# JiaoXianjun/multi-rtl-sdr-calibration

Hardware: AMD Instinct MI355X
Metric: IQ Msamples/s through FCCH+SCH calib (higher is better)
Workload: dtype f64; 1 GPU; cfg4 full chain gsm_sync_demod.m:107-124: 64 dongle streams (64/GPU) x 1020000 IQ samples (102 frames), fir1(46), FCCH+SCH+total_ppm_calculation, table on the host; streams_per_gpu=64, streams_total=64, output=table, collective=none, rows_checked_vs_oracle_per_rank=0

## Files before the change

### multi-rtl-sdr-calibration_amd/csrc/abi_calls.h

```cpp
#pragma once

const char* gsmcal_version(void) { return GSMCAL_VERSION; }

void gsmcal_params_default(gsmcal_params* p) {
    if (!p) return;
    p->coarse_th_db = 10.0; p->coarse_mv_factor = 10; p->coarse_max_offset = 5; p->min_hits = 5;
    p->fine_max_offset = 64; p->fine_max_ppm = 4000.0; p->fine_gate_snr_db = 5.0; p->fine_noise_bw_hz = 200e3;
    p->sch_max_offset = 8; p->sch_max_ppm = 400.0; p->post_min_bcch = 4;
    p->scan_min_hits = 3; p->scan_spacing = 12500.0; p->scan_spacing_idle = 12500.0 + 1250.0; p->scan_tol = 50.0;
}

int gsmcal_set_params(gsmcal_ctx* c, const gsmcal_params* p) {
    if (!c || !p) return GSMCAL_E_ARG;
    RET_IF(pipe_join(c));
    gsmcal_params d;
    gsmcal_params_default(&d);
    if (p->coarse_mv_factor != d.coarse_mv_factor || p->coarse_max_offset != d.coarse_max_offset ||
        p->fine_max_offset != d.fine_max_offset || p->fine_noise_bw_hz != d.fine_noise_bw_hz || p->sch_max_offset != d.sch_max_offset) {
        c->err = "gsmcal_set_params: a geometry field differs from its default";
        return GSMCAL_E_UNSUPPORTED;
    }
    if (p->min_hits < 2 || p->min_hits > GSMCAL_MAX_HITS || p->scan_min_hits < 1 || p->post_min_bcch < 0) {
        c->err = "gsmcal_set_params: min_hits outside 2..GSMCAL_MAX_HITS, scan_min_hits < 1 or post_min_bcch < 0";
        return GSMCAL_E_ARG;
// ... 41 lines not shown
    (void)hipFuncSetAttribute((const void*)k_burst_tone<1, 0, 0>, hipFuncAttributeMaxDynamicSharedMemorySize, 159 * 1024);
    (void)hipFuncSetAttribute((const void*)k_window_sch<0, 0, 0>, hipFuncAttributeMaxDynamicSharedMemorySize, 159 * 1024);
    (void)hipFuncSetAttribute((const void*)k_post_chain_r<0, 0, 0>, hipFuncAttributeMaxDynamicSharedMemorySize, 159 * 1024);
    (void)hipFuncSetAttribute((const void*)k_post_chain_r<8, 512, 47>, hipFuncAttributeMaxDynamicSharedMemorySize, 159 * 1024);
    (void)hipFuncSetAttribute((const void*)k_sch_equalise, hipFuncAttributeMaxDynamicSharedMemorySize, 159 * 1024);
    (void)hipFuncSetAttribute((const void*)k_sch_fd_training, hipFuncAttributeMaxDynamicSharedMemorySize, 159 * 1024);
    (void)hipFuncSetAttribute((const void*)k_fcch_demod, hipFuncAttributeMaxDynamicSharedMemorySize, 159 * 1024);
    (void)hipFuncSetAttribute((const void*)k_fft_burst<0>, hipFuncAttributeMaxDynamicSharedMemorySize, 159 * 1024);
    (void)hipFuncSetAttribute((const void*)k_fft_burst<1>, hipFuncAttributeMaxDynamicSharedMemorySize, 159 * 1024);
    (void)hipFuncSetAttribute((const void*)k_burst_tone<0, 8, 47>, hipFuncAttributeMaxDynamicSharedMemorySize, 159 * 1024);
    (void)hipFuncSetAttribute((const void*)k_burst_tone<1, 8, 47>, hipFuncAttributeMaxDynamicSharedMemorySize, 159 * 1024);
    (void)hipFuncSetAttribute((const void*)k_window_sch<8, 512, 47>, hipFuncAttributeMaxDynamicSharedMemorySize, 159 * 1024);
    (void)hipGetLastError();
    gsmcal_ctx* c = new gsmcal_ctx();
    gsmcal_params_default(&c->params);
    c->device = device_id;
    c->stream = (hipStream_t)hip_stream;
    c->own_stream = false;
    c->lanes[0].stream = c->stream;
    c->cur = &c->lanes[0];
    const char* e = getenv("GSMCAL_LANES");
    if (e && atoi(e) >= 1) c->n_lanes_cfg = atoi(e) > MAX_LANES ? MAX_LANES : atoi(e);
    { int ncu = 0; if (hipDeviceGetAttribute(&ncu, hipDeviceAttributeMultiprocessorCount, c->device) == hipSuccess && ncu > 0) c->n_cu = ncu; }
    if (const char* e2 = getenv("GSMCAL_SNR_INLINE_MIN")) c->snr_inline_min = atoi(e2);
    if (const char* e2 = getenv("GSMCAL_SNR_INLINE_KEEP")) c->snr_inline_keep = atoi(e2);
    if (const char* e2 = getenv("GSMCAL_FRONT_NT")) c->front_nt = atoi(e2);
    if (const char* e2 = getenv("GSMCAL_SCAN_SPLIT")) c->scan_split = atoi(e2);
    const char* sst = getenv("GSMCAL_SCAN_STAGES");
    if (sst && atoi(sst) >= 1) c->scan_stages = atoi(sst);
    const char* lm = getenv("GSMCAL_LANE_MIN");
    if (lm && atoi(lm) >= 1) c->lane_min = atoi(lm);
    const char* ce = getenv("GSMCAL_CERT");
    if (ce) c->certify = atoi(ce) != 0;
    const char* sfe = getenv("GSMCAL_SNR_FULL");
    if (sfe) c->snr_full = atoi(sfe) != 0;
    const char* sse = getenv("GSMCAL_SNR_SCREEN_DB");
    if (sse) c->snr_screen_db = atof(sse);
    const char* fge = getenv("GSMCAL_FUSE_GATHER");
    if (fge) c->fuse_fine_gather = atoi(fge) != 0;
    const char* fpe = getenv("GSMCAL_FUSE_POST");
    if (fpe) c->fuse_post = atoi(fpe) != 0;
    const char* pse = getenv("GSMCAL_POST_SLOTS");
    if (pse && atoi(pse) >= 1) c->post_slots_cap = atoi(pse);
    const char* pe = getenv("GSMCAL_PRESCREEN");
    if (pe && atoi(pe) == 0) c->prescreen = false;
    const char* fg = getenv("GSMCAL_FRONT_GENERIC");
// ... 1261 lines not shown
```

### multi-rtl-sdr-calibration_amd/csrc/host_plan.h

```cpp
#pragma once
namespace {

struct DevBuf {
    void* p = nullptr;
    size_t cap = 0;
};

struct ProfRec {
    int name_id;
    hipEvent_t e0, e1;
};

}

#define MAX_LANES 32
struct Lane {
    hipStream_t stream = nullptr;
    DevBuf state, dec, win, peaks, snrbuf, x0, chunkrec, openlist, cert, partial, tailctr, xch, xepoch;
    int npartial = 0;
    hipEvent_t done = nullptr;
    hipEvent_t front_done = nullptr;
    int lo = 0, n = 0;
    long snr_stride = 0, snr_nmove = 0;
    int win_l0_len = 0, win_l0_H = 0;
// ... 8 lines not shown
    Lane lanes[MAX_LANES];
    Lane* cur = nullptr;
    int n_lanes_cfg = 4;
    int n_lanes_used = 1;
    const double* cf_lane = nullptr;
    hipEvent_t fork = nullptr;
    struct GraphSlot {
        std::vector<uintptr_t> key;
        unsigned long epoch = 0;
        int seen = 0;
        hipGraph_t graph = nullptr;
        hipGraphExec_t exec = nullptr;
        unsigned long used = 0;
        int fused_streams = 0;
    };
    static constexpr int GRAPH_SLOTS = 4;
    GraphSlot g_calib[GRAPH_SLOTS], g_scan[GRAPH_SLOTS];
    unsigned long g_stamp = 0;
    unsigned long ws_epoch = 0;
    bool use_graph = true;
    bool graph_always = false;
    bool prescreen = true;
    int n_cu = 256;
    int snr_inline_min = 1;
    int snr_inline_keep = 0;
    int front_nt = -1;
    size_t call_raw_bytes = 0;
    const void* last_raw = nullptr;
    bool call_raw_fresh = false;
    int scan_split = 88;
    int scan_stages = 0;
    int lane_min = 64;
    bool certify = true;
    bool snr_full = true;
    double snr_screen_db = 5.0;
    bool fuse_fine_gather = true;
    static constexpr int FUSED_MAX_STREAMS = 1024;
    std::vector<unsigned> fused_expected;
    unsigned* fused_done = nullptr;
    int fused_hi = 0;
    unsigned long long n_fused_launches = 0, n_gate_fallbacks = 0;
    int capture_fused_streams = 0;
    struct FusedCall {
        const uint8_t* d_raw; int d; long n; int ntaps, len_ts;
        std::vector<double> coef, ts, cf;
        double* d_table; double* d_pos_info; double* d_r_correct; long* d_r_len;
// ... 185 lines not shown
    int kind;
    const uint8_t* raw; long raw_stride;
    const cplx* arr; long arr_stride;
    const double* coef; int ntaps;
};

size_t gather_lds(int len, int level, int kind, int ntaps, bool to_lds = false) {
    return gather_carve(len, level, kind, ntaps, to_lds).total;
}

GatherArgs gather_args(const Source& src, int level, int len) {
    GatherArgs a;
    memset(&a, 0, sizeof(a));
    a.src_kind = src.kind; a.level = level; a.len = len; a.tiles = 0; a.ntaps = src.ntaps;
    a.raw = src.raw; a.raw_stride = src.raw_stride; a.arr = src.arr; a.arr_stride = src.arr_stride;
    a.coef = src.coef;
    return a;
}

size_t fused_lds(const Source& src, int level, int len, size_t scratch, bool compact_xs = false) {
    return (gather_carve(len, level, src.kind, src.ntaps, true, compact_xs).total + scratch + 15) & ~(size_t)15;
}

int launch_gather(gsmcal_ctx* c, int S, const Source& src, int level, int len, bool tiles, int nwin_grid,
                  cplx* dst, long dst_stream_stride, long dst_win_stride) {
    GatherArgs a;
    memset(&a, 0, sizeof(a));
    a.src_kind = src.kind; a.level = level; a.len = len; a.tiles = tiles ? 1 : 0; a.ntaps = src.ntaps; a.pad = 0;
    a.raw = src.raw; a.raw_stride = src.raw_stride; a.arr = src.arr; a.arr_stride = src.arr_stride;
    a.coef = src.coef; a.dst = dst; a.dst_stream_stride = dst_stream_stride; a.dst_win_stride = dst_win_stride;
    const size_t lds = gather_lds(len, level, src.kind, src.ntaps);
    LAUNCH(c, k_gather, dim3(nwin_grid, S), dim3(256), lds, (const StreamState*)c->cur->state.p, a);
    CHECK_LAUNCH(c);
    return 0;
}

int ensure_twiddles(gsmcal_ctx* c, int nfft) {
    if (c->tw_n == nfft) return 0;
    RET_IF(ensure(c, c->tw, (size_t)nfft * sizeof(cplx)));
    LAUNCH(c, k_make_twiddles, dim3((nfft + 255) / 256), dim3(256), 0, (cplx*)c->tw.p, nfft);
    CHECK_LAUNCH(c);
    c->tw_n = nfft;
    ++c->ws_epoch;
    return 0;
}

// ... 279 lines not shown
                return 0;
            }
        }
        TailArgs tl;
        RET_IF(make_tail(c, S, sa_fine, STEP_FINE_DECIDE, lvl, 0, tl));
        LAUNCH(c, k_fine_verify, dim3(H, S), dim3(FV_THREADS), vlds, (const StreamState*)st, (const cplx*)win, sstride, wstride,
               g.fine_nshift, g.nfft, (const cplx*)c->tw.p, (const ChunkRec*)c->cur->chunkrec.p, peaks, H, certp, n_open,
               st, tl);
    } else {
        RET_IF(ensure(c, c->cur->x0, (size_t)S * H * g.nfft * sizeof(cplx)));
        LAUNCH(c, k_fft_burst<1>, dim3(H, S), dim3(FFT_THREADS), fft_lds(g), (const StreamState*)st, (const cplx*)win, sstride,
               wstride, g.nfft, (const cplx*)c->tw.p, (PeakOut*)nullptr, (cplx*)c->cur->x0.p, H);
        LAUNCH(c, k_fine_search, dim3(g.NB, H, S), dim3(256), (size_t)(g.fine_nshift - 1 + FS_CHUNK) * sizeof(cplx),
               (const StreamState*)st, (const cplx*)win, sstride, wstride, g.fine_nshift, g.nfft, (const cplx*)c->cur->x0.p,
               peaks, H, g.NB);
        LAUNCH(c, k_step<STEP_FINE_DECIDE>, dim3(S), dim3(64), 0, st, sa_fine, lvl, 0);
    }
    {
        GatherArgs ga = gather_args(src, lvl + 1, g.nfft);
        if (c->cur->win_l0_len > 0) { ga.l0 = win; ga.l0_stream_stride = sstride; ga.l0_win_stride = wstride; ga.l0_len = c->cur->win_l0_len; }
        TailArgs tl;
        RET_IF(make_tail(c, S, sa, next_sch_lvl >= 0 ? (STEP_CARRIER_DECIDE | STEP_SCH_SETUP) : STEP_CARRIER_DECIDE, lvl,
                         next_sch_lvl >= 0 ? next_sch_lvl : 0, tl));
        LAUNCH_GEOM(g.ov == 8 && src.kind == SRC_RAW && src.ntaps == 47 && lvl == 0, c, (k_burst_tone<1, 8, 47>), (k_burst_tone<1, 0, 0>), dim3(H, S), dim3(BT_THREADS), fused_lds(src, lvl + 1, g.nfft, burst_scratch(g)), st, ga,
               g.nfft, (const cplx*)c->tw.p, g.ov, 1, tl);
    }
    CHECK_LAUNCH(c);
    return 0;
}

int run_sch(gsmcal_ctx* c, int S, const Source& src, int lvl, const Geom& g, int H, int len_ts, bool setup_done,
            int next_post_lvl) {
    StreamState* st = (StreamState*)c->cur->state.p;
    const int wl = g.sch_nshift - 1 + len_ts;
    const long wstride = g.fine_wlen > wl ? g.fine_wlen : wl, sstride = (long)H * wstride;
    RET_IF(ensure(c, c->cur->win, (size_t)S * sstride * sizeof(cplx)));
    const StepArgs sa = step_args(c, g, H, len_ts);
    if (!setup_done) LAUNCH(c, k_step<STEP_SCH_SETUP>, dim3(S), dim3(64), 0, st, sa, 0, lvl);
    {
        const GatherArgs ga = gather_args(src, lvl, wl);
        const size_t scratch = (size_t)(len_ts + g.sch_nshift * SCH_PARTS) * sizeof(cplx) + (size_t)g.sch_nshift * sizeof(double);
        TailArgs tl;
        RET_IF(make_tail(c, S, sa, next_post_lvl >= 0 ? (STEP_SCH_DECIDE | STEP_POST_SETUP) : STEP_SCH_DECIDE, lvl,
                         next_post_lvl >= 0 ? next_post_lvl : 0, tl));
        LAUNCH_GEOM(g.ov == 8 && len_ts == 512 && src.kind == SRC_RAW && src.ntaps == 47 && lvl == 2, c, (k_window_sch<8, 512, 47>), (k_window_sch<0, 0, 0>), dim3(H, S), dim3(512), fused_lds(src, lvl, wl, scratch), st, ga, (const cplx*)c->ts.p,
               len_ts, g.sch_nshift, tl);
    }
    CHECK_LAUNCH(c);
    return 0;
}

int run_post(gsmcal_ctx* c, int S, const Source& src, int lvl, const Geom& g, int H, bool setup_done, double* table,
             double* pos_info_out, long* r_len_out) {
    StreamState* st = (StreamState*)c->cur->state.p;
    const long wstride = g.fine_wlen, sstride = (long)H * g.fine_wlen;
    RET_IF(ensure(c, c->cur->win, (size_t)S * sstride * sizeof(cplx)));
    RET_IF(ensure(c, c->cur->peaks, (size_t)S * H * g.NB * sizeof(PeakOut)));
    RET_IF(ensure_twiddles(c, g.nfft));
    cplx* win = (cplx*)c->cur->win.p;
    StepArgs sa = step_args(c, g, H, 0);
    sa.table = table; sa.pos_info_out = pos_info_out; sa.r_len_out = r_len_out;
    if (!setup_done) LAUNCH(c, k_step<STEP_POST_SETUP>, dim3(S), dim3(64), 0, st, sa, 0, lvl);
    {
        GatherArgs ga = gather_args(src, lvl, g.nfft);
        if (c->cur->win_l0_len == g.fine_wlen && c->cur->win_l0_H == H && src.kind == SRC_RAW) {
            ga.l0 = win; ga.l0_stream_stride = sstride; ga.l0_win_stride = wstride; ga.l0_len = c->cur->win_l0_len;
        }
        TailArgs tl;
        RET_IF(make_tail(c, S, sa, table ? (STEP_POST_DECIDE | STEP_TOTALS) : STEP_POST_DECIDE, lvl, 0, tl));
        LAUNCH_GEOM(g.ov == 8 && src.kind == SRC_RAW && src.ntaps == 47 && lvl == 3, c, (k_burst_tone<0, 8, 47>), (k_burst_tone<0, 0, 0>), dim3(H, S), dim3(BT_THREADS), fused_lds(src, lvl, g.nfft, burst_scratch(g)), st, ga,
               g.nfft, (const cplx*)c->tw.p, g.ov, 0, tl);
    }
    CHECK_LAUNCH(c);
    return 0;
}

int init_states(gsmcal_ctx* c, int S, long n0) {
    (void)n0;
    RET_IF(ensure(c, c->cur->state, (size_t)S * sizeof(StreamState)));
    HIPCHK(c, hipMemsetAsync(c->cur->state.p, 0, (size_t)S * sizeof(StreamState), c->cur->stream));
    c->last_S = S;
    return 0;
}

int dc_means(gsmcal_ctx* c, const uint8_t* d_raw, int S, long n) {
    int blocks = (int)((2 * n / 16 + 256 * 8 - 1) / (256 * 8));
    if (blocks < 1) blocks = 1;
    int cap = 4096 / (S > 0 ? S : 1);
    if (cap < 1) cap = 1;
    if (blocks > cap) blocks = cap;
    LAUNCH(c, k_dc_sum, dim3(blocks, S), dim3(256), 0, d_raw, 2 * n, (StreamState*)c->cur->state.p);
    LAUNCH(c, k_finish_mean, dim3((S + 63) / 64), dim3(64), 0, (StreamState*)c->cur->state.p, S, n);
    CHECK_LAUNCH(c);
// ... 419 lines not shown
```

### multi-rtl-sdr-calibration_amd/csrc/kernels_estim.h

```cpp
#pragma once
#include "state.h"
#include "kernels_frontend.h"
#include "kernels_detect.h"

#define GSM_SYMBOL_RATE ((1625.0 / 6.0) * 1e3)
#define TWO_PI_D (2.0 * 3.14159265358979323846)
#define PI_D 3.14159265358979323846

__device__ __forceinline__ PeakOut merge_peaks(const PeakOut* p, int NB) {
    PeakOut b = p[0];
    for (int i = 1; i < NB; ++i)
        if (p[i].p > b.p || (p[i].p == b.p && p[i].tie < b.tie)) b = p[i];
    return b;
}

__device__ __forceinline__ void coherent_store(double* p, double v) {
    __hip_atomic_store(p, v, __ATOMIC_RELAXED, __HIP_MEMORY_SCOPE_AGENT);
}
__device__ __forceinline__ unsigned long long coherent_load(const unsigned long long* p) {
    return __hip_atomic_load(p, __ATOMIC_RELAXED, __HIP_MEMORY_SCOPE_AGENT);
}
__device__ __forceinline__ PeakOut coherent_peak(const PeakOut* p) {
    static_assert(sizeof(PeakOut) == 16, "two 64-bit words");
    const unsigned long long a = coherent_load((const unsigned long long*)p), b = coherent_load((const unsigned long long*)p + 1);
    PeakOut o;
    o.p = __longlong_as_double((long long)a);
    o.tie = (int)(b & 0xffffffffu);
    o.k = (int)(b >> 32);
    return o;
}
__device__ __forceinline__ PeakOut merge_peaks_coherent(const PeakOut* p, int NB) {
    PeakOut b = coherent_peak(p);
    for (int i = 1; i < NB; ++i) {
        const PeakOut q = coherent_peak(p + i);
        if (q.p > b.p || (q.p == b.p && q.tie < b.tie)) b = q;
    }
    return b;
}

#define PCR_PRIO(P0, P1, P2) { const unsigned rnd_ = (blockIdx.y * gridDim.x + blockIdx.x) >> 8; if (rnd_ == 0) __builtin_amdgcn_s_setprio(P0); else if (rnd_ == 1) __builtin_amdgcn_s_setprio(P1); else __builtin_amdgcn_s_setprio(P2); }
#define BT_THREADS 512

__device__ __forceinline__ int uni_i(int v) { return __builtin_amdgcn_readfirstlane(v); }
__device__ __forceinline__ long uni_l(long v) {
    return (long)(((unsigned long long)(unsigned)__builtin_amdgcn_readfirstlane((int)((unsigned long long)v >> 32)) << 32) |
                  (unsigned)__builtin_amdgcn_readfirstlane((int)v));
}
__device__ __forceinline__ double uni_d(double v) { return __longlong_as_double(uni_l(__double_as_longlong(v))); }
template <int NT, int KID = -1>
__device__ __forceinline__ int burst_gather_fast(const StreamState* __restrict__ st, const GatherArgs& a, unsigned char* smem,
                                                 int widx, int s, const cplx* __restrict__ tw_g, int nfft) {
    const int tid = threadIdx.x, level = a.level;
    if (!a.l0 || a.src_kind != SRC_RAW || a.tiles || (level != 1 && level != 3) || nfft > 3 * NT || nfft > a.len + 40) return 0;
    if (widx >= MAXH) return -1;
    typedef const __attribute__((address_space(3))) StreamState* LdsState;
    LdsState sl = (LdsState)st;
    const int lane = tid & 63;
    const int v_nwin = sl->n_win, v_t1 = sl->op[1].type, v_t2 = sl->op[2].type, v_t3 = sl->op[3].type, v_nf = sl->n_fine_ws;
    const double v_f1 = sl->op[1].param, v_c2 = sl->op[2].param, v_f3 = sl->op[3].param;
    const long v_ws = sl->win_start[widx], v_n2 = sl->op[2].n, v_n0 = sl->n0;
    const long fw = lane < MAXH ? sl->fine_ws[lane] : 0;
    if (widx >= uni_i(v_nwin)) return -1;
    if (uni_i(v_t1) != OP_LERP) return 0;
    const double f1 = uni_d(v_f1);
// ... 66 lines not shown
    auto lvl2 = [&](int i) {
        return cmul(buf1[i], cmul(cmul(T[0], T[1 + (i >> 5)]), T[1 + GC_ROT_A + (i & 31)]));
    };
    if (t3 == OP_LERP) {
#pragma unroll 1
        for (int i = tid; i < L; i += NT) {
            const long k = lo3 + i;
            const double xq = lerp_pos((double)k, f3);
            const long i0 = (long)floor(xq);
            const long i1 = i0 + 1 > hi1 ? hi1 : i0 + 1;
            const double t = xq - (double)i0;
            const cplx v0 = lvl2((int)(i0 - lo1)), v1 = lvl2((int)(i1 - lo1));
            buf0[i] = make_double2(v0.x + t * (v1.x - v0.x), v0.y + t * (v1.y - v0.y));
        }
    } else {
        for (int i = tid; i < L; i += NT) buf0[i] = lvl2(i);
    }
    __syncthreads();
    if (tid < nfft) buf1[tid] = tw0;
    if (tid + NT < nfft) buf1[tid + NT] = tw1;
    if (tid + 2 * NT < nfft) buf1[tid + 2 * NT] = tw2;
    return 1;
}
#define BT_STAMP(i) DEV_STAMP(GATE ? KID_BT1 : KID_BT0, blockIdx.y * gridDim.x + blockIdx.x, i)
template <int GATE, int FIR_UNR = 1>
__device__ __forceinline__ void burst_tone_body(StreamState* __restrict__ sts, const GatherArgs& a, int nfft,
                                                const cplx* __restrict__ tw_g, int ov, int prior_mode,
                                                unsigned char* smem, double* res = nullptr,
                                                bool state_in_lds = false) {
    __shared__ double red_p[BT_THREADS / 64];
    __shared__ int red_t[BT_THREADS / 64];
    __shared__ double red[2 * (BT_THREADS / 64)];
    __shared__ double sh_phase;
    __shared__ int sh_key;
    const int s = blockIdx.y, w = blockIdx.x, tid = threadIdx.x;
    BT_STAMP(0);
    const int fast = state_in_lds ? burst_gather_fast<BT_THREADS, GATE ? KID_BT1 : KID_BT0>(sts + s, a, smem, w, s, tw_g, nfft) : 0;
    if (fast < 0) return;
    cplx* xs = (cplx*)smem;
    if (!fast) {
        xs = gather_core<BT_THREADS, GATE ? KID_BT1 : KID_BT0, FIR_UNR>(sts, a, smem, w, s, true);
        if (!xs) return;
        __syncthreads();
    }
    BT_STAMP(1);
    StreamState* st = sts + s;
    const int N2 = nfft / 37, ldb = N2 + 1;
    const GatherCarve gc = gather_carve(a.len, a.level, a.src_kind, a.ntaps, true, a.pad != 0);
    cplx* B = (xs == (cplx*)smem) ? (cplx*)(smem + gc.off_region1) : (cplx*)smem;
    cplx* w37 = (cplx*)(smem + gc.total);
    cplx* wN2 = w37 + 40;
    double* P = (double*)(wN2 + N2);
    cplx* twl = B;
    if (!fast) for (int n = tid; n < nfft; n += BT_THREADS) twl[n] = tw_g[n];
    fft37_tables(w37, wN2, N2, tid, tw_g);
    __syncthreads();
    {
        double e = 0.0;
        for (int n = tid; n < nfft; n += BT_THREADS) { const cplx v = xs[n]; e = fma(v.x, v.x, fma(v.y, v.y, e)); }
        e = wave_sum(e);
        if ((tid & 63) == 0) red[tid >> 6] = e;
        const int wave = tid >> 6, lane = tid & 63;
        const int prior = prior_mode == 1 ? st_i32(&st->prior_bin[w]) : nfft / 32;
        if (wave < 7) {
            int k = prior - 3 + wave;
            k = ((k % nfft) + nfft) % nfft;
            double ar = 0.0, ai = 0.0;
            int idx = (int)(((unsigned)k * (unsigned)lane) % (unsigned)nfft);
            const int stp = (int)(((unsigned)k * 64u) % (unsigned)nfft);
// ... 67 lines not shown
        auto pass = [&](const cplx* tw) {
            for (int n = tid; n < nfft - 1; n += BT_THREADS) {
                const unsigned i0 = ((unsigned)n * jm) % (unsigned)nfft;
                const unsigned i1 = i0 + jm >= (unsigned)nfft ? i0 + jm - (unsigned)nfft : i0 + jm;
                const cplx ub = unit(cmul(xs[n], tw[i0]));
                const cplx ua = unit(cmul(xs[n + 1], tw[i1]));
                sr += ua.x * ub.x + ua.y * ub.y;
                si += ua.y * ub.x - ua.x * ub.y;
            }
        };
        if (full) pass(tw_g); else pass(twl);
    }
    sr = wave_sum(sr);
    si = wave_sum(si);
    if ((tid & 63) == 0) { red[2 * (tid >> 6)] = sr; red[2 * (tid >> 6) + 1] = si; }
    __syncthreads();
    if (tid == 0) {
        double tr = 0.0, ti = 0.0;
        for (int i = 0; i < BT_THREADS / 64; ++i) { tr += red[2 * i]; ti += red[2 * i + 1]; }
        const double cnt = (double)(nfft - 1);
        const double phase = atan2(ti / cnt, tr / cnt);
        sh_phase = phase;
        const double fo = sampling_rate * (ipr + phase) / TWO_PI_D;
        if (res) res[0] = fo; else coherent_store(&st->fo_burst[w], fo);
    }
    BT_STAMP(3);
    if (!GATE) return;
    if (state_in_lds) PCR_PRIO(0, 1, 2)
    __syncthreads();
    const double phase = sh_phase;
    cplx* pw = (cplx*)P;
    cplx* base = pw + 16;
    if (tid < 16) {
        double sn, cs;
        sincos((double)tid * phase, &sn, &cs);
        pw[tid] = make_double2(cs, -sn);
    } else if (tid >= 64 && tid < 64 + (nfft + 15) / 16) {
        double sn, cs;
        sincos((double)((tid - 64) * 16) * phase, &sn, &cs);
        base[tid - 64] = make_double2(cs, -sn);
    }
    __syncthreads();
    if (full) {
        fft37_step1_sym<true>(xs, B, w37, tw_g, nfft, N2, ldb, tid, BT_THREADS, [&](int n, const cplx& v) {
            return cmul(cmul(v, tw_g[((unsigned)n * jm) % (unsigned)nfft]), cmul(base[n >> 4], pw[n & 15])); });
    } else {
        fft37_step1_sym<true>(xs, B, w37, tw_g, nfft, N2, ldb, tid, BT_THREADS, [&](int n, const cplx& v) {
            return cmul(cmul(v, twl[((unsigned)n * jm) % (unsigned)nfft]), cmul(base[n >> 4], pw[n & 15])); });
    }
    __syncthreads();
    const int hnl = (int)ceil(((double)nfft * 200e3 / sampling_rate) / 2.0);
    const int nb = 2 * hnl;
    for (int b = tid; b < nb; b += BT_THREADS) {
        const int k = b < hnl ? b : nfft - nb + b;
        const cplx X = fft37_step2_bin(B, wN2, N2, ldb, k);
        const double m = hypot(X.x, X.y);
        P[b] = m * m;
    }
    __syncthreads();
    if (tid < 64) {
        double noi = 0.0;
        for (int k = 3 + tid; k < nb - 2; k += 64) noi += P[k];
        noi = wave_sum(noi);
        if (tid == 0) {
            double sig = 0.0;
            for (int k = 0; k < 3; ++k) sig += P[k];
            for (int k = nb - 2; k < nb; ++k) sig += P[k];
            const double sn = 10.0 * log10(sig / noi);
            if (res) res[1] = sn; else coherent_store(&st->snr_burst[w], sn);
        }
    }
    BT_STAMP(4);
}

#define SCH_PARTS 4
template <int NSH, int LT>
__device__ __forceinline__ void sch_corr_rows(cplx* __restrict__ xs_w, const cplx* __restrict__ ts, cplx* __restrict__ tcp,
                                              double* __restrict__ cv, int tid, int nthreads) {
    constexpr int R = 4, Q = 16, M = 39;
    constexpr int NG = (NSH + R - 1) / R, PADL = R * NG, NTC = PADL + Q * M, WL = NSH - 1 + LT;
    static_assert(Q * M >= WL && Q * M <= WL + 40, "the stretches cover the window and stay inside the gather buffer's slack");
    for (int i = tid; i < NTC; i += nthreads) {
        const int n = i - PADL;
        tcp[i] = (n >= 0 && n < LT) ? make_double2(ts[n].x, -ts[n].y) : make_double2(0.0, 0.0);
    }
    for (int i = WL + tid; i < Q * M; i += nthreads) xs_w[i] = make_double2(0.0, 0.0);
    __syncthreads();
    if (tid < NG * Q) {
        const int g = tid >> 4, q = tid & 15;
        const cplx* __restrict__ xp = xs_w + q * M;
        const cplx* __restrict__ tp = tcp + PADL + q * M - R * g;
        cplx T1 = tp[-1], T2 = tp[-2], T3 = tp[-3];
// ... 8 lines not shown
            SCH_STEP(s + 1, T3, T0, T1, T2)
            SCH_STEP(s + 2, T2, T3, T0, T1)
            SCH_STEP(s + 3, T1, T2, T3, T0)
        }
        static_assert(M % 4 == 3, "three samples left");
        SCH_STEP(s, T0, T1, T2, T3)
        SCH_STEP(s + 1, T3, T0, T1, T2)
        SCH_STEP(s + 2, T2, T3, T0, T1)
#undef SCH_STEP
#undef SCH_MAC
#define SCH_ROWSUM(V) V += dpp_move_f64<0xB1, 0xF>(V); V += dpp_move_f64<0x4E, 0xF>(V); V += dpp_move_f64<0x141, 0xF>(V); V += dpp_move_f64<0x140, 0xF>(V);
        SCH_ROWSUM(ar0) SCH_ROWSUM(ai0) SCH_ROWSUM(ar1) SCH_ROWSUM(ai1) SCH_ROWSUM(ar2) SCH_ROWSUM(ai2) SCH_ROWSUM(ar3) SCH_ROWSUM(ai3)
#undef SCH_ROWSUM
        const double sr = q == 0 ? ar0 : (q == 1 ? ar1 : (q == 2 ? ar2 : ar3)), si = q == 0 ? ai0 : (q == 1 ? ai1 : (q == 2 ? ai2 : ai3));
        const int o = R * g + q;
        if (q < R && o < NSH) {
            const double m = hypot(sr, si);
            cv[o] = m * m;
        }
    }
    __syncthreads();
}

template <int FIR_UNR = 1, bool FAST = false>
__device__ __forceinline__ void window_sch_body(StreamState* __restrict__ sts, const GatherArgs& a,
                                                const cplx* __restrict__ ts, int len_ts, int nshift,
                                                unsigned char* smem, double* res = nullptr) {
    const int s = blockIdx.y, w = blockIdx.x, tid = threadIdx.x;
    DEV_STAMP(KID_SCH, blockIdx.y * gridDim.x + blockIdx.x, 0);
    cplx* xs = gather_core<512, -1, FIR_UNR>(sts, a, smem, w, s, true);
    if (!xs) return;
    DEV_STAMP(KID_SCH, blockIdx.y * gridDim.x + blockIdx.x, 1);
    const GatherCarve gc = gather_carve(a.len, a.level, a.src_kind, a.ntaps, true, a.pad != 0);
    cplx* tc = (cplx*)(smem + gc.total);
    cplx* part = tc + len_ts;
    double* cv = (double*)(part + nshift * SCH_PARTS);
    __syncthreads();
    StreamState* st = sts + s;
    if (FAST) {
        sch_corr_rows<89, 512>(xs, ts, tc, cv, tid, 512);
    } else {
    for (int i = tid; i < len_ts; i += 512) tc[i] = make_double2(ts[i].x, -ts[i].y);
    __syncthreads();
    const int seg = (len_ts + SCH_PARTS - 1) / SCH_PARTS;
    const int full = (nshift * SCH_PARTS / 512) * (512 / SCH_PARTS);
    const int n_task_sh = (full > 0 && nshift - full <= 2) ? full : nshift;
    __shared__ double rest[2][2 * 8];
    for (int t = tid; t < n_task_sh * SCH_PARTS; t += 512) {
        const int o = t % n_task_sh, q = t / n_task_sh;
        const int n0 = q * seg, n1 = n0 + seg < len_ts ? n0 + seg : len_ts;
        double ar = 0.0, ai = 0.0;
#pragma unroll 8
        for (int n = n0; n < n1; ++n) {
            const cplx c = tc[n], v = xs[o + n];
            ar = fma(c.x, v.x, fma(-c.y, v.y, ar));
            ai = fma(c.x, v.y, fma(c.y, v.x, ai));
        }
        part[q * nshift + o] = make_double2(ar, ai);
    }
    for (int o = n_task_sh; o < nshift; ++o) {
        double ar = 0.0, ai = 0.0;
// ... 15 lines not shown
            for (int q = 0; q < 8; ++q) { ar += rest[o - n_task_sh][2 * q]; ai += rest[o - n_task_sh][2 * q + 1]; }
        }
        const double m = hypot(ar, ai);
        cv[o] = m * m;
    }
    __syncthreads();
    }
    DEV_STAMP(KID_SCH, blockIdx.y * gridDim.x + blockIdx.x, 2);
    if (tid < 64) {
        int mi = 0x7fffffff;
        double mx = -1.0;
        for (int o = tid; o < nshift; o += 64)
            if (cv[o] > mx) { mx = cv[o]; mi = o; }
        for (int off = 32; off > 0; off >>= 1) {
            const double om = __shfl_down(mx, off, 64);
            const int oi = __shfl_down(mi, off, 64);
            if (om > mx || (om == mx && oi < mi)) { mx = om; mi = oi; }
        }
        if (tid == 0) {
            const double sp = (double)(st_i64(&st->win_start[w]) + 1 + mi);
            const bool edge = mi == 0 || mi == nshift - 1;
            if (res) { res[0] = sp; res[1] = edge ? 1.0 : 0.0; }
            else {
                coherent_store(&st->sch_first[w], sp);
                if (edge) atomicOr(&st->sch_edge, 1);
            }
        }
    }
}

__device__ __forceinline__ void wsync() {
    __builtin_amdgcn_fence(__ATOMIC_ACQ_REL, "wavefront");
    __builtin_amdgcn_wave_barrier();
}
#define LANE0(...) do { if (lane == 0) { __VA_ARGS__; } } while (0)
__device__ __forceinline__ unsigned long long bits_below(int n) { return n >= 64 ? ~0ull : ((1ull << n) - 1ull); }

__device__ __forceinline__ void fine_sentinel(StreamState* st) {
    st->n_fcch = 0; st->fcch_is_sentinel = 1;
    st->sampling_ppm1 = INFINITY; st->carrier_ppm1 = INFINITY;
    st->r1_kind = 0; st->n_win = 0; st->n_fine = 0; st->n_fine_ws = 0;
}

__device__ void d_fine_setup(StreamState* st, int ov, int lvl, int min_hits, int lane) {
    LANE0(fine_sentinel(st));
    if (lane >= 1 && lane < NLEVELS && lane > lvl) { st->op[lane].type = OP_NONE; st->op[lane].n = 0; }
    if (st->status < 0) return;
    if (st->n_coarse < min_hits) { LANE0(set_status(st, 0, GSMCAL_S_FEW_HITS)); return; }
// ... 371 lines not shown
__device__ __forceinline__ void stream_tail(StreamState* __restrict__ sts, const TailArgs& t, unsigned char* smem, int kid = -1) {
    if (!t.ctr) return;
    __shared__ int sh_last;
    __builtin_amdgcn_fence(__ATOMIC_RELEASE, "workgroup");
    __builtin_amdgcn_s_waitcnt(0);
    __syncthreads();
    if (threadIdx.x == 0) {
        const unsigned old = atomicAdd(&t.ctr[blockIdx.y], 1u);
        sh_last = old == gridDim.x - 1;
        if (sh_last) atomicExch(&t.ctr[blockIdx.y], 0u);
    }
    __syncthreads();
    if (!sh_last) return;
    step_body<true>(sts, t.sa, t.steps, t.lvl_a, t.lvl_b, blockIdx.y, (StreamState*)smem, kid);
}

template <int GATE, int OV, int NTAPS>
__global__ void __launch_bounds__(BT_THREADS) __attribute__((amdgpu_waves_per_eu(6, 8)))
k_burst_tone(StreamState* __restrict__ sts, GatherArgs a_in, int nfft_rt, const cplx* __restrict__ tw_g, int ov_rt, int prior_mode,
             TailArgs tail) {
    extern __shared__ __attribute__((aligned(16))) unsigned char smem[];
    GatherArgs a = a_in;
    const int nfft = OV > 0 ? 148 * OV : nfft_rt, ov = OV > 0 ? OV : ov_rt;
    if (OV > 0) { a.len = 148 * OV; a.ntaps = NTAPS; a.src_kind = SRC_RAW; a.tiles = 0; a.level = GATE ? 1 : 3; }
    burst_tone_body<GATE, (OV > 0 ? 2 : 1)>(sts, a, nfft, tw_g, ov, prior_mode, smem);
    DEV_STAMP(GATE ? KID_BT1 : KID_BT0, blockIdx.y * gridDim.x + blockIdx.x, 5);
    stream_tail(sts, tail, smem, GATE ? KID_BT1 : KID_BT0);
    DEV_STAMP(GATE ? KID_BT1 : KID_BT0, blockIdx.y * gridDim.x + blockIdx.x, 6);
}

template <int OV, int LT, int NTAPS>
__global__ void __launch_bounds__(512) __attribute__((amdgpu_waves_per_eu(6, 8))) k_window_sch(StreamState* __restrict__ sts, GatherArgs a_in,
                                                    const cplx* __restrict__ ts, int len_ts_rt, int nshift_rt, TailArgs tail) {
    extern __shared__ __attribute__((aligned(16))) unsigned char smem[];
    GatherArgs a = a_in;
    const int len_ts = OV > 0 ? LT : len_ts_rt, nshift = OV > 0 ? 11 * OV + 1 : nshift_rt;
    if (OV > 0) { a.len = 11 * OV + LT; a.ntaps = NTAPS; a.src_kind = SRC_RAW; a.tiles = 0; a.level = 2; }
    window_sch_body<(OV > 0 ? 2 : 1), (OV == 8 && LT == 512)>(sts, a, ts, len_ts, nshift, smem);
    DEV_STAMP(KID_SCH, blockIdx.y * gridDim.x + blockIdx.x, 3);
    stream_tail(sts, tail, smem, KID_SCH);
    DEV_STAMP(KID_SCH, blockIdx.y * gridDim.x + blockIdx.x, 4);
}

__global__ void __launch_bounds__(FV_THREADS) k_fine_verify(const StreamState* __restrict__ sts,
                                                     const cplx* __restrict__ win, long win_stream_stride,
                                                     long win_stride, int nshift, int nfft,
                                                     const cplx* __restrict__ tw_g, const ChunkRec* __restrict__ rec,
                                                     PeakOut* __restrict__ out, int H,
                                                     const FineCert* __restrict__ cert, int* __restrict__ n_open,
                                                     StreamState* __restrict__ sts_rw, TailArgs tail) {
    extern __shared__ __attribute__((aligned(16))) unsigned char smem[];
    DEV_STAMP(KID_VERIFY, blockIdx.y * gridDim.x + blockIdx.x, 0);
    fine_verify_body<FV_THREADS>(sts, win, win_stream_stride, win_stride, nshift, nfft, tw_g, rec, out, H, cert, n_open, smem);
    DEV_STAMP(KID_VERIFY, blockIdx.y * gridDim.x + blockIdx.x, 1);
    stream_tail(sts_rw, tail, smem, KID_VERIFY);
    DEV_STAMP(KID_VERIFY, blockIdx.y * gridDim.x + blockIdx.x, 2);
}

#define PC_THREADS 512
struct PostChainArgs {
    GatherArgs ga1, ga_sch, ga0;
    StepArgs sa;
    unsigned* done;
    unsigned* timed_out;
    unsigned long long poll_ticks;
    int test_stall;
    int lvl_fine, lvl_sch, lvl_post;
    int nfft, ov, len_ts, sch_nshift, fine_nshift, H;
    const cplx* tw_g; const cplx* ts;
    const cplx* win; long win_stream_stride, win_stride;
    const ChunkRec* rec; const FineCert* cert; PeakOut* peaks; int* n_open;
    int with_totals, pad;
};

#define PCR_EMPTY 0xFFFFFFFFFFFFFFFFull
#define PCR_STATE_BYTES ((sizeof(StreamState) + 15) & ~(size_t)15)

__device__ __forceinline__ unsigned long long pcr_word(double v) {
    return v != v ? 0x7FF8000000000000ull : (unsigned long long)__double_as_longlong(v);
}

__device__ __forceinline__ void pcr_exchange(unsigned long long* __restrict__ slots, int H, int w, unsigned long long r0,
                                             unsigned long long r1, unsigned long long* all, StreamState* sh, bool collect,
                                             unsigned long long poll_ticks, unsigned* __restrict__ timed_out, bool publish = true) {
    const int tid = threadIdx.x;
    if (tid < 2 && publish) __hip_atomic_store(slots + 2 * w + tid, tid ? r1 : r0, __ATOMIC_RELAXED, __HIP_MEMORY_SCOPE_AGENT);
    if (!collect) return;
    if (tid < 64) {
        const bool mine = tid < 2 * H;
        unsigned long long v = PCR_EMPTY;
        unsigned spins = 0;
        unsigned long long t0 = 0;
        bool bad = false;
        while (true) {
            if (mine && v == PCR_EMPTY) v = __hip_atomic_load(slots + tid, __ATOMIC_RELAXED, __HIP_MEMORY_SCOPE_AGENT);
            if (!__ballot(mine && v == PCR_EMPTY)) break;
            __builtin_amdgcn_s_sleep(4);
            if ((++spins & 255u) == 0u) {
                const unsigned long long now = wall_clock64();
// ... 130 lines not shown
```

Measured before the change: 515,300 Msample/s.

## Stage per-stream state in LDS and add fast SCH gather for specialized tail kernels

The specialized burst-tone and SCH window kernels now copy the per-stream StreamState into LDS at entry and read it from there, writing results back to the global state. A new sch_gather_fast path fuses raw u8 IQ loading, FIR, lerp resampling and mixing using LDS-resident state. It is used only when the combined LDS footprint lets three blocks fit on a CU, with a fallback to the generic kernels otherwise. The aim is to cut repeated global state reads and gather overhead, at the cost of extra LDS per block and possibly lower occupancy.

```diff
diff --git a/multi-rtl-sdr-calibration_amd/csrc/abi_calls.h b/multi-rtl-sdr-calibration_amd/csrc/abi_calls.h
--- a/multi-rtl-sdr-calibration_amd/csrc/abi_calls.h
+++ b/multi-rtl-sdr-calibration_amd/csrc/abi_calls.h
@@ -87,6 +87,7 @@
     const char* e = getenv("GSMCAL_LANES");
     if (e && atoi(e) >= 1) c->n_lanes_cfg = atoi(e) > MAX_LANES ? MAX_LANES : atoi(e);
     { int ncu = 0; if (hipDeviceGetAttribute(&ncu, hipDeviceAttributeMultiprocessorCount, c->device) == hipSuccess && ncu > 0) c->n_cu = ncu; }
+    { int lds = 0; if (hipDeviceGetAttribute(&lds, hipDeviceAttributeMaxSharedMemoryPerMultiprocessor, c->device) == hipSuccess && lds > 0) c->lds_per_cu = (size_t)lds; }
     if (const char* e2 = getenv("GSMCAL_SNR_INLINE_MIN")) c->snr_inline_min = atoi(e2);
     if (const char* e2 = getenv("GSMCAL_SNR_INLINE_KEEP")) c->snr_inline_keep = atoi(e2);
     if (const char* e2 = getenv("GSMCAL_FRONT_NT")) c->front_nt = atoi(e2);
diff --git a/multi-rtl-sdr-calibration_amd/csrc/host_plan.h b/multi-rtl-sdr-calibration_amd/csrc/host_plan.h
--- a/multi-rtl-sdr-calibration_amd/csrc/host_plan.h
+++ b/multi-rtl-sdr-calibration_amd/csrc/host_plan.h
@@ -54,6 +54,7 @@
     bool graph_always = false;
     bool prescreen = true;
     int n_cu = 256;
+    size_t lds_per_cu = 160 * 1024;
     int snr_inline_min = 1;
     int snr_inline_keep = 0;
     int front_nt = -1;
@@ -285,6 +286,12 @@
     return (gather_carve(len, level, src.kind, src.ntaps, true, compact_xs).total + scratch + 15) & ~(size_t)15;
 }
 
+#define LEAN_TAIL_STATIC_LDS 1536
+size_t lean_tail_lds(const gsmcal_ctx* c, const Source& src, int level, int len, size_t scratch, bool compact_xs) {
+    const size_t lds = fused_lds(src, level, len, scratch, compact_xs) + PCR_STATE_BYTES;
+    return (lds <= 159 * 1024 && 3 * (lds + LEAN_TAIL_STATIC_LDS) <= c->lds_per_cu) ? lds : 0;
+}
+
 int launch_gather(gsmcal_ctx* c, int S, const Source& src, int level, int len, bool tiles, int nwin_grid,
                   cplx* dst, long dst_stream_stride, long dst_win_stride) {
     GatherArgs a;
@@ -610,7 +617,8 @@
         TailArgs tl;
         RET_IF(make_tail(c, S, sa, next_sch_lvl >= 0 ? (STEP_CARRIER_DECIDE | STEP_SCH_SETUP) : STEP_CARRIER_DECIDE, lvl,
                          next_sch_lvl >= 0 ? next_sch_lvl : 0, tl));
-        LAUNCH_GEOM(g.ov == 8 && src.kind == SRC_RAW && src.ntaps == 47 && lvl == 0, c, (k_burst_tone<1, 8, 47>), (k_burst_tone<1, 0, 0>), dim3(H, S), dim3(BT_THREADS), fused_lds(src, lvl + 1, g.nfft, burst_scratch(g)), st, ga,
+        const size_t lean = (g.ov == 8 && src.kind == SRC_RAW && src.ntaps == 47 && lvl == 0) ? lean_tail_lds(c, src, lvl + 1, g.nfft, burst_scratch(g), true) : 0;
+        LAUNCH_GEOM(lean > 0, c, (k_burst_tone<1, 8, 47>), (k_burst_tone<1, 0, 0>), dim3(H, S), dim3(BT_THREADS), lean > 0 ? lean : fused_lds(src, lvl + 1, g.nfft, burst_scratch(g)), st, ga,
                g.nfft, (const cplx*)c->tw.p, g.ov, 1, tl);
     }
     CHECK_LAUNCH(c);
@@ -631,7 +639,8 @@
         TailArgs tl;
         RET_IF(make_tail(c, S, sa, next_post_lvl >= 0 ? (STEP_SCH_DECIDE | STEP_POST_SETUP) : STEP_SCH_DECIDE, lvl,
                          next_post_lvl >= 0 ? next_post_lvl : 0, tl));
-        LAUNCH_GEOM(g.ov == 8 && len_ts == 512 && src.kind == SRC_RAW && src.ntaps == 47 && lvl == 2, c, (k_window_sch<8, 512, 47>), (k_window_sch<0, 0, 0>), dim3(H, S), dim3(512), fused_lds(src, lvl, wl, scratch), st, ga, (const cplx*)c->ts.p,
+        const size_t lean = (g.ov == 8 && len_ts == 512 && src.kind == SRC_RAW && src.ntaps == 47 && lvl == 2) ? lean_tail_lds(c, src, lvl, wl, scratch, false) : 0;
+        LAUNCH_GEOM(lean > 0, c, (k_window_sch<8, 512, 47>), (k_window_sch<0, 0, 0>), dim3(H, S), dim3(512), lean > 0 ? lean : fused_lds(src, lvl, wl, scratch), st, ga, (const cplx*)c->ts.p,
                len_ts, g.sch_nshift, tl);
     }
     CHECK_LAUNCH(c);
@@ -656,7 +665,8 @@
         }
         TailArgs tl;
         RET_IF(make_tail(c, S, sa, table ? (STEP_POST_DECIDE | STEP_TOTALS) : STEP_POST_DECIDE, lvl, 0, tl));
-        LAUNCH_GEOM(g.ov == 8 && src.kind == SRC_RAW && src.ntaps == 47 && lvl == 3, c, (k_burst_tone<0, 8, 47>), (k_burst_tone<0, 0, 0>), dim3(H, S), dim3(BT_THREADS), fused_lds(src, lvl, g.nfft, burst_scratch(g)), st, ga,
+        const size_t lean = (g.ov == 8 && src.kind == SRC_RAW && src.ntaps == 47 && lvl == 3) ? lean_tail_lds(c, src, lvl, g.nfft, burst_scratch(g), true) : 0;
+        LAUNCH_GEOM(lean > 0, c, (k_burst_tone<0, 8, 47>), (k_burst_tone<0, 0, 0>), dim3(H, S), dim3(BT_THREADS), lean > 0 ? lean : fused_lds(src, lvl, g.nfft, burst_scratch(g)), st, ga,
                g.nfft, (const cplx*)c->tw.p, g.ov, 0, tl);
     }
     CHECK_LAUNCH(c);
diff --git a/multi-rtl-sdr-calibration_amd/csrc/kernels_estim.h b/multi-rtl-sdr-calibration_amd/csrc/kernels_estim.h
--- a/multi-rtl-sdr-calibration_amd/csrc/kernels_estim.h
+++ b/multi-rtl-sdr-calibration_amd/csrc/kernels_estim.h
@@ -40,6 +40,7 @@
 
 #define PCR_PRIO(P0, P1, P2) { const unsigned rnd_ = (blockIdx.y * gridDim.x + blockIdx.x) >> 8; if (rnd_ == 0) __builtin_amdgcn_s_setprio(P0); else if (rnd_ == 1) __builtin_amdgcn_s_setprio(P1); else __builtin_amdgcn_s_setprio(P2); }
 #define BT_THREADS 512
+#define PCR_STATE_BYTES ((sizeof(StreamState) + 15) & ~(size_t)15)
 
 __device__ __forceinline__ int uni_i(int v) { return __builtin_amdgcn_readfirstlane(v); }
 __device__ __forceinline__ long uni_l(long v) {
@@ -152,12 +153,114 @@
     if (tid + 2 * NT < nfft) buf1[tid + 2 * NT] = tw2;
     return 1;
 }
+
+template <int NT, int FIR_UNR = 1>
+__device__ __forceinline__ int sch_gather_fast(const StreamState* __restrict__ st, const GatherArgs& a, unsigned char* smem,
+                                               int widx, int s) {
+    const int tid = threadIdx.x;
+    const int L = a.len;
+    if (a.src_kind != SRC_RAW || a.tiles || a.level != 2 || a.ntaps != 47 || a.pad != 0 || L > 32 * GC_ROT_A) return 0;
+    if (widx >= MAXH) return -1;
+    typedef const __attribute__((address_space(3))) StreamState* LdsState;
+    LdsState sl = (LdsState)st;
+    const int v_nwin = sl->n_win, v_t1 = sl->op[1].type, v_t2 = sl->op[2].type;
+    const double v_f1 = sl->op[1].param, v_c2 = sl->op[2].param, v_mr = sl->mean_re, v_mi = sl->mean_im;
+    const long v_ws = sl->win_start[widx], v_n0 = sl->n0;
+    if (widx >= uni_i(v_nwin)) return -1;
+    if (uni_i(v_t1) != OP_LERP || uni_i(v_t2) != OP_MIX) return 0;
+    const double f1 = uni_d(v_f1), c2 = uni_d(v_c2);
+    const long n0 = uni_l(v_n0);
+    const long lo1 = uni_l(v_ws), hi1 = lo1 + L - 1;
+    const long lo0 = (long)floor((double)lo1 * f1);
+    long hi0 = (long)floor((double)hi1 * f1) + 1;
+    hi0 = hi0 > n0 - 1 ? n0 - 1 : hi0;
+    if (hi0 < lo0 || hi0 - lo0 + 1 > (long)L + 8) return 0;
+    const int cnt0 = (int)(hi0 - lo0 + 1);
+    const GatherCarve gc = gather_carve(L, 2, SRC_RAW, a.ntaps, true, false);
+    cplx* buf0 = (cplx*)smem;
+    cplx* buf1 = (cplx*)(smem + gc.off_region1);
+    cplx* xs = buf1;
+    double* c_s = (double*)(smem + gc.off_coef);
+    cplx* T = (cplx*)(smem + gc.off_rot);
+    const unsigned short* base = (const unsigned short*)(a.raw + (size_t)s * a.raw_stride);
+    const int ntp = a.ntaps;
+    const long first = lo0 - (ntp - 1);
+    const int span = cnt0 + ntp - 1;
+    const long ao = (long)(((uintptr_t)base >> 1) & 7);
+    long m = (first + ao) % 8;
+    if (m < 0) m += 8;
+    const long first_al = first - m;
+    const int nchunk = (int)((m + span + 8 + 7) >> 3);
+    const int nwc = (nchunk + 63) >> 6;
+    if (nchunk > NT - 128) return 0;
+    if (tid < 64 * nwc) {
+        uint4 v = make_uint4(0, 0, 0, 0);
+        const long g0 = first_al + 8L * tid;
+        if (tid < nchunk) {
+            if (g0 >= 0 && g0 + 8 <= n0) {
+                v = *(const uint4*)(base + g0);
+            } else {
+                unsigned short t[8];
+#pragma unroll
+                for (int i = 0; i < 8; ++i) t[i] = (g0 + i >= 0 && g0 + i < n0) ? base[g0 + i] : (unsigned short)0;
+                v.x = t[0] | ((unsigned)t[1] << 16); v.y = t[2] | ((unsigned)t[3] << 16);
+                v.z = t[4] | ((unsigned)t[5] << 16); v.w = t[6] | ((unsigned)t[7] << 16);
+            }
+            const double mr = uni_d(v_mr), mi = uni_d(v_mi);
+            const int i_base = 8 * tid - (int)m;
+            const unsigned wv[4] = {v.x, v.y, v.z, v.w};
+#pragma unroll
+            for (int u = 0; u < 8; ++u) {
+                const int i = i_base + u;
+                const long g = g0 + u;
+                const unsigned q = (wv[u >> 1] >> (16 * (u & 1))) & 0xFFFFu;
+                cplx x = make_double2(0.0, 0.0);
+                if (i < span && g >= 0 && g < n0) x = make_double2((double)(q & 0xFF) - mr, (double)(q >> 8) - mi);
+                if (i >= 0 && i < span + 8) xs[xs_pad(i)] = x;
+            }
+        }
+    } else {
+        const int t = tid - 64 * nwc, nh = NT - 64 * nwc;
+        const int na = (L + 31) >> 5;
+        if (t >= 64) fir_stage_taps(c_s, a.coef, ntp, t - 64, nh - 64);
+        else {
+            for (int i = t; i < 1 + na + 32; i += 64) {
+                const double arg = i == 0 ? (double)lo1 * c2 : (i <= na ? (double)(32 * (i - 1)) * c2 : (double)(i - 1 - na) * c2);
+                double sn, cs;
+                sincos_large(arg, &sn, &cs);
+                T[i == 0 ? 0 : (i <= na ? i : 1 + GC_ROT_A + (i - 1 - na))] = make_double2(cs, sn);
+            }
+        }
+    }
+    __syncthreads();
+    for (int i0 = 4 * tid; i0 < cnt0; i0 += 4 * NT) {
+        cplx y0, y1, y2, y3;
+        fir4_lds<0, true, FIR_UNR>(xs, c_s, i0, ntp, &y0, &y1, &y2, &y3);
+        buf0[i0] = y0;
+        if (i0 + 1 < cnt0) buf0[i0 + 1] = y1;
+        if (i0 + 2 < cnt0) buf0[i0 + 2] = y2;
+        if (i0 + 3 < cnt0) buf0[i0 + 3] = y3;
+    }
+    __syncthreads();
+    for (int i = tid; i < L; i += NT) {
+        const long k = lo1 + i;
+        const double xq = lerp_pos((double)k, f1);
+        const long i0 = (long)floor(xq);
+        const long i1 = i0 + 1 > hi0 ? hi0 : i0 + 1;
+        const double t = xq - (double)i0;
+        const cplx v0 = buf0[i0 - lo0], v1 = buf0[i1 - lo0];
+        const cplx l1 = make_double2(v0.x + t * (v1.x - v0.x), v0.y + t * (v1.y - v0.y));
+        buf1[i] = cmul(l1, cmul(cmul(T[0], T[1 + (i >> 5)]), T[1 + GC_ROT_A + (i & 31)]));
+    }
+    return 1;
+}
 #define BT_STAMP(i) DEV_STAMP(GATE ? KID_BT1 : KID_BT0, blockIdx.y * gridDim.x + blockIdx.x, i)
-template <int GATE, int FIR_UNR = 1>
+template <int GATE, int FIR_UNR = 1, bool LEAN = false>
 __device__ __forceinline__ void burst_tone_body(StreamState* __restrict__ sts, const GatherArgs& a, int nfft,
                                                 const cplx* __restrict__ tw_g, int ov, int prior_mode,
                                                 unsigned char* smem, double* res = nullptr,
-                                                bool state_in_lds = false) {
+                                                bool state_in_lds = false,
+                                                StreamState* __restrict__ st_out = nullptr) {
     __shared__ double red_p[BT_THREADS / 64];
     __shared__ int red_t[BT_THREADS / 64];
     __shared__ double red[2 * (BT_THREADS / 64)];
@@ -165,7 +268,7 @@
     __shared__ int sh_key;
     const int s = blockIdx.y, w = blockIdx.x, tid = threadIdx.x;
     BT_STAMP(0);
-    const int fast = state_in_lds ? burst_gather_fast<BT_THREADS, GATE ? KID_BT1 : KID_BT0>(sts + s, a, smem, w, s, tw_g, nfft) : 0;
+    const int fast = (LEAN || state_in_lds) ? burst_gather_fast<BT_THREADS, GATE ? KID_BT1 : KID_BT0>(sts + s, a, smem, w, s, tw_g, nfft) : 0;
     if (fast < 0) return;
     cplx* xs = (cplx*)smem;
     if (!fast) {
@@ -175,6 +278,7 @@
     }
     BT_STAMP(1);
     StreamState* st = sts + s;
+    StreamState* sto = LEAN ? st_out + s : st;
     const int N2 = nfft / 37, ldb = N2 + 1;
     const GatherCarve gc = gather_carve(a.len, a.level, a.src_kind, a.ntaps, true, a.pad != 0);
     cplx* B = (xs == (cplx*)smem) ? (cplx*)(smem + gc.off_region1) : (cplx*)smem;
@@ -288,7 +392,7 @@
         const double phase = atan2(ti / cnt, tr / cnt);
         sh_phase = phase;
         const double fo = sampling_rate * (ipr + phase) / TWO_PI_D;
-        if (res) res[0] = fo; else coherent_store(&st->fo_burst[w], fo);
+        if (res) res[0] = fo; else coherent_store(&sto->fo_burst[w], fo);
     }
     BT_STAMP(3);
     if (!GATE) return;
@@ -333,7 +437,7 @@
             for (int k = 0; k < 3; ++k) sig += P[k];
             for (int k = nb - 2; k < nb; ++k) sig += P[k];
             const double sn = 10.0 * log10(sig / noi);
-            if (res) res[1] = sn; else coherent_store(&st->snr_burst[w], sn);
+            if (res) res[1] = sn; else coherent_store(&sto->snr_burst[w], sn);
         }
     }
     BT_STAMP(4);
@@ -388,13 +492,17 @@
     __syncthreads();
 }
 
-template <int FIR_UNR = 1, bool FAST = false>
+template <int FIR_UNR = 1, bool FAST = false, bool LEAN = false>
 __device__ __forceinline__ void window_sch_body(StreamState* __restrict__ sts, const GatherArgs& a,
                                                 const cplx* __restrict__ ts, int len_ts, int nshift,
-                                                unsigned char* smem, double* res = nullptr) {
+                                                unsigned char* smem, double* res = nullptr,
+                                                StreamState* __restrict__ st_out = nullptr) {
     const int s = blockIdx.y, w = blockIdx.x, tid = threadIdx.x;
     DEV_STAMP(KID_SCH, blockIdx.y * gridDim.x + blockIdx.x, 0);
-    cplx* xs = gather_core<512, -1, FIR_UNR>(sts, a, smem, w, s, true);
+    const int fast = LEAN ? sch_gather_fast<512, FIR_UNR>(sts + s, a, smem, w, s) : 0;
+    if (fast < 0) return;
+    cplx* xs = fast ? (cplx*)(smem + gather_carve(a.len, a.level, a.src_kind, a.ntaps, true, a.pad != 0).off_region1)
+                    : gather_core<512, -1, FIR_UNR>(sts, a, smem, w, s, true);
     if (!xs) return;
     DEV_STAMP(KID_SCH, blockIdx.y * gridDim.x + blockIdx.x, 1);
     const GatherCarve gc = gather_carve(a.len, a.level, a.src_kind, a.ntaps, true, a.pad != 0);
@@ -403,6 +511,7 @@
     double* cv = (double*)(part + nshift * SCH_PARTS);
     __syncthreads();
     StreamState* st = sts + s;
+    StreamState* sto = LEAN ? st_out + s : st;
     if (FAST) {
         sch_corr_rows<89, 512>(xs, ts, tc, cv, tid, 512);
     } else {
@@ -464,8 +573,8 @@
             const bool edge = mi == 0 || mi == nshift - 1;
             if (res) { res[0] = sp; res[1] = edge ? 1.0 : 0.0; }
             else {
-                coherent_store(&st->sch_first[w], sp);
-                if (edge) atomicOr(&st->sch_edge, 1);
+                coherent_store(&sto->sch_first[w], sp);
+                if (edge) atomicOr(&sto->sch_edge, 1);
             }
         }
     }
@@ -883,8 +992,19 @@
     extern __shared__ __attribute__((aligned(16))) unsigned char smem[];
     GatherArgs a = a_in;
     const int nfft = OV > 0 ? 148 * OV : nfft_rt, ov = OV > 0 ? OV : ov_rt;
-    if (OV > 0) { a.len = 148 * OV; a.ntaps = NTAPS; a.src_kind = SRC_RAW; a.tiles = 0; a.level = GATE ? 1 : 3; }
-    burst_tone_body<GATE, (OV > 0 ? 2 : 1)>(sts, a, nfft, tw_g, ov, prior_mode, smem);
+    if (OV > 0) {
+        a.len = 148 * OV; a.ntaps = NTAPS; a.src_kind = SRC_RAW; a.tiles = 0; a.level = GATE ? 1 : 3; a.pad = 1;
+        StreamState* sh = (StreamState*)smem;
+        {
+            const uint4* src = (const uint4*)(sts + blockIdx.y);
+            uint4* dst = (uint4*)sh;
+            for (int i = threadIdx.x; i < (int)(sizeof(StreamState) / 16); i += BT_THREADS) dst[i] = src[i];
+        }
+        __syncthreads();
+        burst_tone_body<GATE, 2, true>(sh - blockIdx.y, a, nfft, tw_g, ov, prior_mode, smem + PCR_STATE_BYTES, nullptr, false, sts);
+    } else {
+        burst_tone_body<GATE, 1>(sts, a, nfft, tw_g, ov, prior_mode, smem);
+    }
     DEV_STAMP(GATE ? KID_BT1 : KID_BT0, blockIdx.y * gridDim.x + blockIdx.x, 5);
     stream_tail(sts, tail, smem, GATE ? KID_BT1 : KID_BT0);
     DEV_STAMP(GATE ? KID_BT1 : KID_BT0, blockIdx.y * gridDim.x + blockIdx.x, 6);
@@ -896,8 +1016,19 @@
     extern __shared__ __attribute__((aligned(16))) unsigned char smem[];
     GatherArgs a = a_in;
     const int len_ts = OV > 0 ? LT : len_ts_rt, nshift = OV > 0 ? 11 * OV + 1 : nshift_rt;
-    if (OV > 0) { a.len = 11 * OV + LT; a.ntaps = NTAPS; a.src_kind = SRC_RAW; a.tiles = 0; a.level = 2; }
-    window_sch_body<(OV > 0 ? 2 : 1), (OV == 8 && LT == 512)>(sts, a, ts, len_ts, nshift, smem);
+    if (OV > 0) {
+        a.len = 11 * OV + LT; a.ntaps = NTAPS; a.src_kind = SRC_RAW; a.tiles = 0; a.level = 2; a.pad = 0;
+        StreamState* sh = (StreamState*)smem;
+        {
+            const uint4* src = (const uint4*)(sts + blockIdx.y);
+            uint4* dst = (uint4*)sh;
+            for (int i = threadIdx.x; i < (int)(sizeof(StreamState) / 16); i += 512) dst[i] = src[i];
+        }
+        __syncthreads();
+        window_sch_body<2, (OV == 8 && LT == 512), true>(sh - blockIdx.y, a, ts, len_ts, nshift, smem + PCR_STATE_BYTES, nullptr, sts);
+    } else {
+        window_sch_body<1, false>(sts, a, ts, len_ts, nshift, smem);
+    }
     DEV_STAMP(KID_SCH, blockIdx.y * gridDim.x + blockIdx.x, 3);
     stream_tail(sts, tail, smem, KID_SCH);
     DEV_STAMP(KID_SCH, blockIdx.y * gridDim.x + blockIdx.x, 4);
@@ -935,7 +1066,6 @@
 };
 
 #define PCR_EMPTY 0xFFFFFFFFFFFFFFFFull
-#define PCR_STATE_BYTES ((sizeof(StreamState) + 15) & ~(size_t)15)
 
 __device__ __forceinline__ unsigned long long pcr_word(double v) {
     return v != v ? 0x7FF8000000000000ull : (unsigned long long)__double_as_longlong(v);
```

New measurement: 533,400 Msample/s (median of 6 runs). +3.5%, better.
